# JGCRI/xanthos

Measured on AMD Instinct MI355X. Metric: cell-months/sec (pm_abcd_mrtm, 67,420 cells), higher is better.
Workload: dtype f64

## Files before the change

### xanthos_amd/csrc/xh_fused.hip

```cpp
#include <algorithm>
#include <string>

#include "xh_mrtm_flow.h"
#include "xh_stage.h"

namespace {

int fused_resources(xh_ctx *ctx, size_t n_events) {
    if (!ctx->side_stream[0]) {
        int least = 0, greatest = 0;
        XH_HIP(ctx, hipDeviceGetStreamPriorityRange(&least, &greatest));
        const int prio = least != 0 ? least : greatest;
        ctx->feed_queue_ok = least != greatest;
        XH_HIP(ctx, hipStreamCreateWithPriority(&ctx->side_stream[0], hipStreamNonBlocking, prio));
        if (xh_flow_debug()) fprintf(stderr, "[libxanthos_hip] side stream priority %d (range %d .. %d)\n", prio, least, greatest);
    }
    while (ctx->side_events.size() < n_events) {
        hipEvent_t e = nullptr;
        XH_HIP(ctx, hipEventCreateWithFlags(&e, hipEventDisableTiming));
        ctx->side_events.push_back(e);
    }
    return XH_OK;
}

__global__ void k_set_word(unsigned *w, unsigned v) {
    if (threadIdx.x == 0) __hip_atomic_store(w, v, __ATOMIC_RELAXED, __HIP_MEMORY_SCOPE_AGENT);
}

__global__ void k_gate(unsigned *w, unsigned epoch, unsigned long long limit_ticks) {
    if (threadIdx.x != 0) return;
    const unsigned long long t0 = __builtin_amdgcn_s_memrealtime();
    while ((int)(__hip_atomic_fetch_add(w, 0u, __ATOMIC_RELAXED, __HIP_MEMORY_SCOPE_AGENT) - epoch) < 0) {
        if (__builtin_amdgcn_s_memrealtime() - t0 > limit_ticks) break;
        __builtin_amdgcn_s_sleep(32);
    }
}

int run_fed(xh_ctx *ctx, const xh_fused_args *a, xh_pm_setup &pm, xh_abcd_setup &ab, bool *runoff_done) {
    *runoff_done = false;
    const int nmonths = a->nmonths;
    int b0 = (std::max(a->abcd_spinup, a->routing_spinup) + 15) & ~15;
    {
        const long long need = (12ll * nmonths - 33ll * a->routing_spinup) * 5 / (45 * 4);
        b0 = std::max(b0, (int)((std::max(need, 0ll) + 15) & ~15ll));
    }
    b0 = std::max(b0, 32);
    hipStream_t A = ctx->stream, B = ctx->side_stream[0];
    auto pm_block = [&](hipStream_t st, int m0, int m1) {
        return xh_pm_enqueue(ctx, st, pm, m0, m1 - m0, a->d_tas, a->d_tmin, a->d_rhs, a->d_wind, a->d_rsds, a->d_rlds, a->d_tairprev,
                             a->d_lct, a->d_elev, a->d_pet);
    };
    auto sim_block = [&](hipStream_t st, int m0, int m1, double *staged) {
        return xh_abcd_enqueue_sim(ctx, st, ab, m0, m1, a->d_pars, a->d_pet, a->d_precip, a->d_abcd_tmin, a->d_aet, a->d_q,
                                   a->d_sav, staged);
    };
    if (nmonths - b0 < 64) return XH_ERR_LIMIT;
    if (!ctx->feed_queue_ok || ctx->feed_disabled) return XH_ERR_LIMIT;
    const size_t lines = (size_t)(nmonths + 15) / 16;
    const size_t need = lines * (size_t)a->ncell * 128 + 256;
    if (need > ctx->feed_bytes) {
        int rc = xh_settle(ctx);
        if (rc) return rc;
        if (ctx->d_feed) XH_HIP(ctx, hipFree(ctx->d_feed));
        ctx->d_feed = nullptr;
        ctx->feed_bytes = 0;
        XH_HIP(ctx, hipMalloc(&ctx->d_feed, need));
        ctx->feed_bytes = need;
        XH_HIP(ctx, hipMemsetAsync(ctx->d_feed, 0, 256, A));
    }
    unsigned *w_ready = static_cast<unsigned *>(ctx->d_feed), *w_epoch = w_ready + 32;
    double *staged = reinterpret_cast<double *>(static_cast<char *>(ctx->d_feed) + 256);
    hipEvent_t ev_blk0 = ctx->side_events[0], ev_done = ctx->side_events[1];

    int rc;
    rc = pm_block(A, 0, b0);
    if (rc) return rc;
    rc = xh_abcd_enqueue_spinup(ctx, A, ab, a->d_pars, a->d_pet, a->d_precip, a->d_abcd_tmin);
    if (rc) return rc;
    rc = sim_block(A, 0, b0, staged);
    if (rc) return rc;
    XH_HIP(ctx, hipEventRecord(ev_blk0, A));
    FlowFeed feed;
    feed.q_staged = staged;
    feed.ncell = a->ncell;
    feed.months_ready = w_ready;
    feed.ready_at_launch = (unsigned)b0;
    feed.place_epoch = w_epoch;
    feed.epoch = ++ctx->feed_epoch;
    rc = xh_route_series_fed(ctx, a->plan, nmonths, a->routing_spinup, a->h_ndays, a->dt, a->d_flow_dist, a->d_velocity,
                             a->d_area, a->d_q, a->d_S0, a->d_chstorage, a->d_avgchflow, a->route_flags, &feed);
    if (rc == XH_ERR_LIMIT) {
        rc = pm_block(A, b0, nmonths);
        if (rc) return rc;
        rc = sim_block(A, b0, nmonths, nullptr);
        *runoff_done = rc == XH_OK;
        return rc ? rc : XH_ERR_LIMIT;
    }
    if (rc) return rc;
    std::string first_error;
    auto rest = [&]() -> int {
        XH_HIP(ctx, hipStreamWaitEvent(B, ev_blk0, 0));
        constexpr unsigned long long gate_ticks = 20000ull * 100ull;
        {
            xh_span sp = xh_span_begin_on(ctx, "feed_gate", B);
            hipLaunchKernelGGL(k_gate, dim3(1), dim3(64), 0, B, w_epoch, feed.epoch, gate_ticks);
            xh_span_end(sp);
        }
        pm.paired = true;
        pm.block = 64;
        int r = pm_block(B, b0, nmonths);
        pm.paired = false;
        pm.block = 0;
        if (r) return r;
        r = sim_block(B, b0, nmonths, staged);
        if (r) return r;
        hipLaunchKernelGGL(k_set_word, dim3(1), dim3(64), 0, B, w_ready, (unsigned)nmonths);
        XH_HIP(ctx, hipGetLastError());
        return XH_OK;
    };
    rc = rest();
    if (rc) first_error = ctx->err;
    if (!ctx->pending_routes.empty() && ctx->pending_routes.back().plan == a->plan && ctx->pending_routes.back().chs == a->d_chstorage)
        ctx->pending_routes.back().seq_after = ctx->work_seq;
    const hipError_t j1 = hipEventRecord(ev_done, B);
    const hipError_t j2 = j1 == hipSuccess ? hipStreamWaitEvent(A, ev_done, 0) : j1;
    if (j2 != hipSuccess) {
        (void)hipStreamSynchronize(B);
        if (!rc) rc = xh_fail(ctx, XH_ERR_HIP, "xh_run_fused: joining the side stream failed: %s", hipGetErrorString(j2));
    }
    if (!rc) {
        ctx->runoff_event = ev_done;
        ctx->runoff_event_fresh = true;
        ctx->runoff_seq = ctx->work_seq;
    }
    if (rc) {
        unsigned *fault = nullptr;
        if (xh_fault_word(ctx, &fault) == XH_OK) hipLaunchKernelGGL(k_set_word, dim3(1), dim3(64), 0, B, fault, 1u);
        if (!first_error.empty()) ctx->err = first_error;
    }
    return rc;
}

}

extern "C" int xh_run_fused(xh_ctx *ctx, const xh_fused_args *a) {
    if (!ctx) return XH_ERR_ARG;
    XH_REQUIRE(ctx, a, "xh_run_fused: NULL argument");
    XH_REQUIRE(ctx, a->d_tas && a->d_tmin && a->d_rhs && a->d_wind && a->d_rsds && a->d_rlds && a->d_lct && a->d_elev &&
                        a->d_pars && a->d_precip && a->d_pet && a->d_q,
               "xh_run_fused: NULL array (PET and runoff are intermediate results and must be given)");
    XH_REQUIRE(ctx, !a->plan || (a->h_ndays && a->d_flow_dist && a->d_velocity && a->d_area),
               "xh_run_fused: routing needs ndays, flow distance, velocity and area");
    const int nmonths = a->nmonths;
    int block = a->block_months > 0 ? a->block_months : 96;
    XH_REQUIRE(ctx, block % 48 == 0, "xh_run_fused: block_months must be a multiple of 48 (whole years and whole lines)");
    XH_REQUIRE(ctx, nmonths > 0 && nmonths % 12 == 0, "xh_run_fused: nmonths must be whole years (PM runs year by year)");
    XH_REQUIRE(ctx, a->abcd_spinup >= 1 && a->abcd_spinup <= nmonths, "xh_run_fused: abcd_spinup out of range");
    xh_pm_setup pm;
    int rc = xh_pm_prepare(ctx, a->pm, a->ncell, nmonths, a->start_year, a->n_lc_years, a->h_lc_years, a->water_idx,
                           a->snow_idx, &pm);
    if (rc) return rc;
    xh_abcd_setup ab;
    rc = xh_abcd_prepare(ctx, a->ncell, nmonths, a->abcd_spinup, a->n_groups, a->h_basin_index, a->h_par_index,
                         a->npar_rows, &ab);
    if (rc || a->ncell == 0) return rc;
    int nblk = (nmonths + block - 1) / block;
    rc = fused_resources(ctx, (size_t)nblk + 3);
    if (rc) return rc;
    if (a->mode == 1 && a->plan) {
        bool runoff_done = false;
        rc = run_fed(ctx, a, pm, ab, &runoff_done);
        if (rc != XH_ERR_LIMIT) return rc;
        if (runoff_done)
            return xh_route_series(ctx, a->plan, nmonths, a->routing_spinup, a->h_ndays, a->dt, a->d_flow_dist, a->d_velocity,
                                   a->d_area, a->d_q, a->d_S0, a->d_chstorage, a->d_avgchflow, nullptr, nullptr,
                                   a->route_flags);
        if (!ctx->feed_queue_ok || ctx->feed_disabled) {
            block = (nmonths + 47) / 48 * 48;
            nblk = 1;
        }
    }
    hipStream_t A = ctx->stream, B = ctx->side_stream[0];
    hipEvent_t ev_start = ctx->side_events[0], ev_done = ctx->side_events[1];
    hipEvent_t *ev_pm = &ctx->side_events[3];

    auto enqueue = [&]() -> int {
        XH_HIP(ctx, hipEventRecord(ev_start, A));
        XH_HIP(ctx, hipStreamWaitEvent(B, ev_start, 0));
        for (int k = 0; k < nblk; ++k) {
            const int m0 = k * block, cnt = std::min(block, nmonths - m0);
            int r = xh_pm_enqueue(ctx, A, pm, m0, cnt, a->d_tas, a->d_tmin, a->d_rhs, a->d_wind, a->d_rsds, a->d_rlds,
                                  a->d_tairprev, a->d_lct, a->d_elev, a->d_pet);
            if (r) return r;
            XH_HIP(ctx, hipEventRecord(ev_pm[k], A));
        }
        XH_HIP(ctx, hipStreamWaitEvent(B, ev_pm[(a->abcd_spinup - 1) / block], 0));
        int r = xh_abcd_enqueue_spinup(ctx, B, ab, a->d_pars, a->d_pet, a->d_precip, a->d_abcd_tmin);
        if (r) return r;
        for (int k = 0; k < nblk; ++k) {
            const int m0 = k * block, m1 = std::min(nmonths, m0 + block);
            XH_HIP(ctx, hipStreamWaitEvent(B, ev_pm[k], 0));
            r = xh_abcd_enqueue_sim(ctx, B, ab, m0, m1, a->d_pars, a->d_pet, a->d_precip, a->d_abcd_tmin, a->d_aet,
                                    a->d_q, a->d_sav, nullptr);
            if (r) return r;
        }
        XH_HIP(ctx, hipGetLastError());
        return XH_OK;
    };
    rc = enqueue();
    const std::string first_error = rc ? ctx->err : std::string();
    const hipError_t j1 = hipEventRecord(ev_done, B);
    const hipError_t j2 = j1 == hipSuccess ? hipStreamWaitEvent(A, ev_done, 0) : j1;
    if (j2 != hipSuccess) {
        (void)hipStreamSynchronize(B);
        if (!rc) rc = xh_fail(ctx, XH_ERR_HIP, "xh_run_fused: joining the side stream failed: %s", hipGetErrorString(j2));
    }
    if (rc) {
        if (!first_error.empty()) ctx->err = first_error;
        return rc;
    }
    if (a->plan)
        return xh_route_series(ctx, a->plan, nmonths, a->routing_spinup, a->h_ndays, a->dt, a->d_flow_dist, a->d_velocity,
                               a->d_area, a->d_q, a->d_S0, a->d_chstorage, a->d_avgchflow, nullptr, nullptr,
                               a->route_flags);
    return XH_OK;
}
```

Before: 3.456 billion.

## Split fed runoff into multiple pieces with progressive ready-word handover

Replaces the single block of PET and ABCD simulation on the side stream with up to four pieces, computed by a new plan helper. After each piece the ready word is advanced, so routing on the main stream can consume earlier months while later months are still being computed. The initial block size b0 no longer uses the balance formula based on nmonths. A two-piece plan falls back to one piece, and environment knobs cap the piece count or insert a debug hold kernel. The cost is more kernel launches and smaller per-launch work.

```diff
diff --git a/xanthos_amd/csrc/xh_feed_plan.h b/xanthos_amd/csrc/xh_feed_plan.h
--- /dev/null
+++ b/xanthos_amd/csrc/xh_feed_plan.h
@@ -0,0 +1,36 @@
+#pragma once
+
+constexpr int XH_FEED_MAX_PIECES = 4, XH_FEED_MIN_PIECE = 64;
+
+struct xh_feed_plan {
+    int b0;
+    int n;
+    int end[XH_FEED_MAX_PIECES];
+};
+
+inline constexpr int xh_feed_b0(int abcd_spinup, int routing_spinup) {
+    const int s = abcd_spinup > routing_spinup ? abcd_spinup : routing_spinup;
+    const int b = (s + 15) & ~15;
+    return b > 32 ? b : 32;
+}
+
+inline constexpr int xh_feed_piece_nowait(int b0, int routing_spinup) { return (routing_spinup + b0 - 2) & ~15; }
+
+inline constexpr xh_feed_plan xh_feed_plan_make(int nmonths, int abcd_spinup, int routing_spinup,
+                                                int max_pieces = XH_FEED_MAX_PIECES) {
+    if (nmonths <= 0 || abcd_spinup < 0 || routing_spinup < 0 || abcd_spinup > nmonths || routing_spinup > nmonths)
+        return xh_feed_plan{32, 0, {0, 0, 0, 0}};
+    xh_feed_plan p{xh_feed_b0(abcd_spinup, routing_spinup), 0, {0, 0, 0, 0}};
+    if (nmonths - p.b0 < XH_FEED_MIN_PIECE) return p;
+    if (max_pieces > XH_FEED_MAX_PIECES) max_pieces = XH_FEED_MAX_PIECES;
+    if (max_pieces < 1) max_pieces = 1;
+    int P = xh_feed_piece_nowait(p.b0, routing_spinup);
+    if (P < XH_FEED_MIN_PIECE) P = XH_FEED_MIN_PIECE;
+    int e = p.b0;
+    while (e < nmonths) {
+        const bool last = p.n + 1 == max_pieces || nmonths - e - P < XH_FEED_MIN_PIECE;
+        e = last ? nmonths : e + P;
+        p.end[p.n++] = e;
+    }
+    return p;
+}
diff --git a/xanthos_amd/csrc/xh_fused.hip b/xanthos_amd/csrc/xh_fused.hip
--- a/xanthos_amd/csrc/xh_fused.hip
+++ b/xanthos_amd/csrc/xh_fused.hip
@@ -1,6 +1,8 @@
 #include <algorithm>
+#include <cstdlib>
 #include <string>
 
+#include "xh_feed_plan.h"
 #include "xh_mrtm_flow.h"
 #include "xh_stage.h"
 
@@ -36,15 +38,22 @@
     }
 }
 
+__global__ void k_hold(unsigned long long ticks) {
+    if (threadIdx.x != 0) return;
+    const unsigned long long t0 = __builtin_amdgcn_s_memrealtime();
+    while (__builtin_amdgcn_s_memrealtime() - t0 < ticks) __builtin_amdgcn_s_sleep(32);
+}
+
 int run_fed(xh_ctx *ctx, const xh_fused_args *a, xh_pm_setup &pm, xh_abcd_setup &ab, bool *runoff_done) {
     *runoff_done = false;
     const int nmonths = a->nmonths;
-    int b0 = (std::max(a->abcd_spinup, a->routing_spinup) + 15) & ~15;
-    {
-        const long long need = (12ll * nmonths - 33ll * a->routing_spinup) * 5 / (45 * 4);
-        b0 = std::max(b0, (int)((std::max(need, 0ll) + 15) & ~15ll));
-    }
-    b0 = std::max(b0, 32);
+    const char *cap = getenv("XH_FEED_PIECES");
+    const int max_pieces = cap ? std::min(std::max(atoi(cap), 1), XH_FEED_MAX_PIECES) : XH_FEED_MAX_PIECES;
+    xh_feed_plan fp = xh_feed_plan_make(nmonths, a->abcd_spinup, a->routing_spinup, max_pieces);
+    if (!cap && fp.n == 2) fp = xh_feed_plan_make(nmonths, a->abcd_spinup, a->routing_spinup, 1);
+    const int b0 = fp.b0;
+    unsigned long long hold_ticks = 0;
+    if (const char *e = getenv("XH_FEED_HOLD_US")) hold_ticks = (unsigned long long)std::min(std::max(atoi(e), 0), 5000) * 100ull;
     hipStream_t A = ctx->stream, B = ctx->side_stream[0];
     auto pm_block = [&](hipStream_t st, int m0, int m1) {
         return xh_pm_enqueue(ctx, st, pm, m0, m1 - m0, a->d_tas, a->d_tmin, a->d_rhs, a->d_wind, a->d_rsds, a->d_rlds, a->d_tairprev,
@@ -54,7 +63,7 @@
         return xh_abcd_enqueue_sim(ctx, st, ab, m0, m1, a->d_pars, a->d_pet, a->d_precip, a->d_abcd_tmin, a->d_aet, a->d_q,
                                    a->d_sav, staged);
     };
-    if (nmonths - b0 < 64) return XH_ERR_LIMIT;
+    if (fp.n == 0) return XH_ERR_LIMIT;
     if (!ctx->feed_queue_ok || ctx->feed_disabled) return XH_ERR_LIMIT;
     const size_t lines = (size_t)(nmonths + 15) / 16;
     const size_t need = lines * (size_t)a->ncell * 128 + 256;
@@ -106,16 +115,22 @@
             hipLaunchKernelGGL(k_gate, dim3(1), dim3(64), 0, B, w_epoch, feed.epoch, gate_ticks);
             xh_span_end(sp);
         }
-        pm.paired = true;
-        pm.block = 64;
-        int r = pm_block(B, b0, nmonths);
-        pm.paired = false;
-        pm.block = 0;
-        if (r) return r;
-        r = sim_block(B, b0, nmonths, staged);
-        if (r) return r;
-        hipLaunchKernelGGL(k_set_word, dim3(1), dim3(64), 0, B, w_ready, (unsigned)nmonths);
-        XH_HIP(ctx, hipGetLastError());
+        for (int k = 0, m0 = b0; k < fp.n; m0 = fp.end[k++]) {
+            const int m1 = fp.end[k];
+            pm.paired = true;
+            pm.block = 64;
+            int r = pm_block(B, m0, m1);
+            pm.paired = false;
+            pm.block = 0;
+            if (r) return r;
+            r = sim_block(B, m0, m1, staged);
+            if (r) return r;
+            xh_span sp = xh_span_begin_on(ctx, "feed_handover", B);
+            if (hold_ticks) hipLaunchKernelGGL(k_hold, dim3(1), dim3(64), 0, B, hold_ticks);
+            hipLaunchKernelGGL(k_set_word, dim3(1), dim3(64), 0, B, w_ready, (unsigned)m1);
+            xh_span_end(sp);
+            XH_HIP(ctx, hipGetLastError());
+        }
         return XH_OK;
     };
     rc = rest();
```

Result: no change. 3.460 billion, median of 3 (+0.1%).
